# alpha-davidson/TensorBNN

Measured on AMD Instinct MI355X. Metric: leapfrog steps/sec (whole node), higher is better.
Workload: dtype f32

## Files before the change

### tensorbnn_amd/csrc/kernels_fast3.hpp

```cpp
#pragma once
#include <type_traits>
#include "kernels_fast.hpp"

template <int I, int N, class F>
__device__ __forceinline__ void sfor3(F&& f) {
    if constexpr (I < N) { f(std::integral_constant<int, I>{}); sfor3<I + 1, N>(f); }
}
template <class S>
struct F3Cfg : FastCfg<S> {
    using B = FastCfg<S>;
    static constexpr int NF(int l) { return (B::out(l) % 16 == 1 || B::out(l) % 16 == 2) ? B::out(l) % 16 : 0; }
    static constexpr int MTF(int l) { return NF(l) ? B::MT(l) - 1 : B::MT(l); }
    static constexpr int fslot(int l, int f) { return 16 * MTF(l) + 4 * f; }
    static constexpr int funit(int l, int f) { return 16 * MTF(l) + f; }
    static constexpr int NLM3 = MTF(B::NL - 1) == 0 ? B::NL - 1 : B::NL;
    static_assert(NLM3 == B::NLM, "fast3 expects the same MFMA/VALU split of the last layer as fast");
    static constexpr int dw_tiles_plain() { int o = 0; for (int m = 0; m < NLM3; ++m) o += MTF(m) * B::NT(m); return o; }
    static constexpr bool NCF(int l) {
        return dw_tiles_plain() <= 39 && l < NLM3 && B::NT(l) >= 2 && MTF(l) >= 1 && MTF(l) <= 4 && B::in(l) + 1 - 16 * (B::NT(l) - 1) <= 4;
    }
    static constexpr int NTF(int l) { return NCF(l) ? B::NT(l) - 1 : B::NT(l); }
    static constexpr int dwt3(int l) { return MTF(l) * NTF(l) + (NCF(l) ? 2 : 0); }
    static constexpr int dwoff3(int l) { int o = 0; for (int m = 0; m < l && m < NLM3; ++m) o += dwt3(m); return o; }
    static constexpr int dwfr3(int l) { return dwoff3(l) + MTF(l) * NTF(l); }
// ... 1066 lines not shown
    static constexpr bool ENABLED = C::DW3_TILES > 0 && C::EP3_TILES == C::DW3_TILES && C::P() >= 2048 &&
                                    (size_t)DENSE_OFF + P4 <= (size_t)C::LDS3_FLOATS;

    template <int W>
    static constexpr int coop_index(int t) {
        if (!CO::ENABLED) return -1;
        for (int l = 0; l < C::NLM3; ++l)
            if (C::MTF(l) > 0 && W < C::MTF(l))
                for (int nt = 0; nt < C::NTF(l); ++nt)
                    if (t == C::dwoff3(l) + W * C::NTF(l) + nt) return CO::cwoff(l) + nt;
        return -1;
    }

    template <int W, int t = 0>
    static __device__ __forceinline__ void stage(f32x4* st, f32x4 (&own)[KMAX], const f32x4 (&dW)[T], const f32x4 (&dWc)[CO::DWC], int lane) {
        if constexpr (t < C::DW3_TILES) {
            f32x4 v = dW[t];
            constexpr int ci = coop_index<W>(t);
            if constexpr (ci >= 0) v += dWc[ci];
            constexpr int sl = slot(t, W);
            if constexpr (sl >= 0) st[sl * 64 + lane] = v;
            else own[t / FAST_WAVES] = v;
            stage<W, t + 1>(st, own, dW, dWc, lane);
        }
    }
    template <int W, int l = 0>
    static __device__ __forceinline__ void stage_nf_coop(f32x4* st, const f32x4 (&dWc)[CO::DWC], int lane) {
        if constexpr (CO::ENABLED && l < C::NLM3) {
            if constexpr (C::MTF(l) > 0 && W < C::MTF(l) && C::NCF(l)) {
                const int i16 = lane & 15, g = lane >> 4;
                if ((i16 & 3) == 0) st[slot(C::dwfr3(l), W) * 64 + 16 * W + 4 * g + (i16 >> 2)] += dWc[CO::cwoff(l) + C::NTF(l)];
            }
            stage_nf_coop<W, l + 1>(st, dWc, lane);
        }
    }
    template <int W, int t, int c>
    static __device__ __forceinline__ f32x4 cpy(const f32x4* st, const f32x4 (&own)[KMAX], int lane) {
        constexpr int sl = slot(t, c);
        if constexpr (sl >= 0) return st[sl * 64 + lane];
        else return own[t / FAST_WAVES];
    }
    static constexpr int NLd = C::NLM3 > 0 ? C::NLM3 : 1;
    template <int W, int k = 0>
    static __device__ __forceinline__ void tiles_sum(const f32x4* st, const f32x4 (&own)[KMAX], int lane, f32x4 (&sum)[KMAX]) {
        if constexpr (k < KMAX) {
            constexpr int t = FAST_WAVES * k + W;
            if constexpr (t < C::DW3_TILES && nf_index(t < C::DW3_TILES ? t : 0) < 0) {
                const f32x4 c0 = cpy<W, t, 0>(st, own, lane), c1 = cpy<W, t, 1>(st, own, lane), c2 = cpy<W, t, 2>(st, own, lane), c3 = cpy<W, t, 3>(st, own, lane);
                sum[k] = (c0 + c1) + (c2 + c3);
            }
            tiles_sum<W, k + 1>(st, own, lane, sum);
        }
    }
    template <int W, int l = 0>
    static __device__ __forceinline__ void nf_sum(const f32x4* st, const f32x4 (&own)[KMAX], int lane, f32x4 (&nfs)[NLd]) {
        if constexpr (l < C::NLM3) {
            if constexpr (C::NCF(l) && (C::dwfr3(l) & (FAST_WAVES - 1)) == W) {
                constexpr int t = C::dwfr3(l);
                const f32x4 c0 = cpy<W, t, 0>(st, own, lane) + cpy<W, t + 1, 0>(st, own, lane), c1 = cpy<W, t, 1>(st, own, lane) + cpy<W, t + 1, 1>(st, own, lane),
                            c2 = cpy<W, t, 2>(st, own, lane) + cpy<W, t + 1, 2>(st, own, lane), c3 = cpy<W, t, 3>(st, own, lane) + cpy<W, t + 1, 3>(st, own, lane);
                nfs[l] = (c0 + c1) + (c2 + c3);
            }
            nf_sum<W, l + 1>(st, own, lane, nfs);
        }
    }
    template <int W, int l = 0>
    static __device__ __forceinline__ void tiles_out(float* dense, const f32x4 (&sum)[KMAX], const f32x4 (&nfs)[NLd], int lane) {
        if constexpr (l < C::NLM3) {
            constexpr int in = C::in(l), out = C::out(l), MT = C::MTF(l);
            if constexpr (C::NCF(l) && (C::dwfr3(l) & (FAST_WAVES - 1)) == W) {
                const int b = lane >> 2, col = unit_of(in, 16 * (C::NT(l) - 1) + 4 * (lane & 3), true);
                if (b < 4 * MT && col >= 0) {
#pragma unroll
                    for (int r = 0; r < 4; ++r) {
                        const int row = unit_of(out, 4 * b + r, false);
                        if (row >= 0) dense[C::offW(l) + (col < in ? row * in + col : in * out + row)] = nfs[l][r];
                    }
                }
            }
            tiles_out_full<W, l, 0>(dense, sum, lane);
            tiles_out<W, l + 1>(dense, sum, nfs, lane);
        }
    }
    template <int W, int l, int k>
    static __device__ __forceinline__ void tiles_out_full(float* dense, const f32x4 (&sum)[KMAX], int lane) {
        constexpr int in = C::in(l), out = C::out(l), MT = C::MTF(l), NT = C::NTF(l);
        if constexpr (k < MT * NT) {
            constexpr int t = C::dwoff3(l) + k, mt = k / (NT > 0 ? NT : 1), nt = k % (NT > 0 ? NT : 1);
            if constexpr ((t & (FAST_WAVES - 1)) == W) {
                const int cs = 16 * nt + (lane & 15), row0 = 16 * mt + 4 * (lane >> 4);
                const int col = l == 0 ? (cs <= in ? cs : -1) : unit_of(in, cs, true);
                if (col >= 0) {
#pragma unroll
                    for (int r = 0; r < 4; ++r) {
                        const int row = unit_of(out, row0 + r, false);
                        if (row >= 0) dense[C::offW(l) + (col < in ? row * in + col : in * out + row)] = sum[t / FAST_WAVES][r];
                    }
                }
            }
            tiles_out_full<W, l, k + 1>(dense, sum, lane);
        }
    }

    template <int W>
    static __device__ __forceinline__ void run(float* __restrict__ lds, float* __restrict__ slab, const f32x4 (&dW)[T], const f32x4 (&dWc)[CO::DWC],
                                               const float (&FP)[FPd], int tid, int lane) {
        const int i16 = lane & 15, g = lane >> 4;
        f32x4* st = reinterpret_cast<f32x4*>(lds);
        float* lb = lds + ST_FLOATS;
        float* dense = lds + DENSE_OFF;
        f32x4 own[KMAX];
        __syncthreads();
        stage<W>(st, own, dW, dWc, lane);
        stage_nf_coop<W>(st, dWc, lane);
        {
            int o = (W * C::FP_REGS * 4 + g) * 16 + i16;
            asm volatile("" : "+v"(o));
#pragma unroll
            for (int r = 0; r < C::FP_REGS; ++r) lb[o + r * 64] = FP[r];
        }
        if (tid < P4 - C::P()) dense[C::P() + tid] = 0.f;
        __syncthreads();
        TSTAMPO(63);
        f32x4 sum[KMAX], nfs[NLd];
        tiles_sum<W>(st, own, lane, sum);
        nf_sum<W>(st, own, lane, nfs);
        float fv[FringeVals<S, 0>::total()];
        int fd[FringeVals<S, 0>::total()];
        FringeVals<S, 0>::template run<0>(lb, tid, fv, fd);
        TSTAMPO(35);
        tiles_out<W>(dense, sum, nfs, lane);
#pragma unroll
        for (int i = 0; i < FringeVals<S, 0>::total(); ++i) if (fd[i] >= 0) dense[fd[i]] = fv[i];
        TSTAMPO(36);
        __syncthreads();
        TSTAMPO(37);
        {
            constexpr int N4 = P4 / 4, NE = (N4 + FAST_THREADS - 1) / FAST_THREADS;
            f32x4 d[NE];
#pragma unroll
            for (int k = 0; k < NE; ++k) {
                const int e = tid + k * FAST_THREADS;
                d[k] = *reinterpret_cast<const f32x4*>(dense + 4 * (e < N4 ? e : 0));
            }
#pragma unroll
            for (int k = 0; k < NE; ++k) {
                const int e = tid + k * FAST_THREADS;
                if (e < N4) store16<true>(slab + 4 * e, d[k]);
            }
        }
    }
};

__device__ __forceinline__ void lds_dma16(const float* gsrc, float* lbase) {
#if defined(__HIP_DEVICE_COMPILE__)
    __builtin_amdgcn_global_load_lds(gsrc, lbase, 16, 0, 0);
#else
    (void)gsrc; (void)lbase;
#endif
}

template <class S>
__global__ __launch_bounds__(FAST_THREADS, 1) __attribute__((amdgpu_waves_per_eu(1, 1))) void k_fwd_bwd_fast3(
    NetDev nd, const float* __restrict__ qimg, const float* __restrict__ eta,
    const float* __restrict__ X, const float* __restrict__ Y, long n,
    float* __restrict__ slabs, int pitch, double* __restrict__ pstat, unsigned long long* __restrict__ stamps, ChainStride cs)
{
    using C = F3Cfg<S>;
    if (chain_done(cs.ctl, cs.t, blockIdx.y)) return;
    qimg += (size_t)blockIdx.y * cs.img; eta += (size_t)blockIdx.y * cs.eta; slabs += (size_t)blockIdx.y * cs.slab; pstat += (size_t)blockIdx.y * PSTAT_CAP;
    static_assert(C::VL && C::NF(C::NL - 1) == C::out(C::NL - 1) && C::MTF(C::NL - 1) == 0, "fast3: last layer must be all-fringe");
    using CO = Coop3<S>;
    static_assert((C::LDS3_FLOATS + (CO::ENABLED ? 2 * CO::XB : 4)) * 4 + 64 <= 160 * 1024, "LDS budget");
    static_assert((size_t)FAST_WAVES * C::FP_REGS * 64 <= (size_t)C::LDS3_FLOATS, "fringe staging does not fit");
#define TB_STAMP(i) do { if (stamps && threadIdx.x == 0 && blockIdx.x == 0) { stamps[i] = wall_clock64(); stamps[8 + i] = clock64(); } } while (0)
    TB_STAMP(0); TSTAMPO(57);
    __shared__ __attribute__((aligned(16))) float lds[C::LDS3_FLOATS];
    __shared__ __attribute__((aligned(16))) float xch[CO::ENABLED ? 2 * CO::XB : 4];
    __shared__ double red[FAST_WAVES];
    const int tid = threadIdx.x, lane = tid & 63, wave = __builtin_amdgcn_readfirstlane(tid >> 6);
    const int i16 = lane & 15, g = lane >> 4;
    float* wl = lds + C::STATIC_FLOATS + wave * C::WAVE3_FLOATS;
    constexpr int d_in = C::in(0), d_out = C::out(C::NL - 1), L = C::NL - 1;
    const long ntiles = (n + 15) / 16;
    const long W = (long)gridDim.x * FAST_WAVES;
    const long wg = (long)blockIdx.x * FAST_WAVES + wave;
    float xn[C::KS0], yn[d_out], wn = 1.f;
    auto fetch = [&](long tile) {
        const long row = tile * 16 + i16;
        const bool ok = tile < ntiles && row < n;
#pragma unroll
        for (int t = 0; t < C::KS0; ++t) {
            const int u = 4 * t + g;
            xn[t] = (ok && u < d_in) ? X[row * d_in + u] : 0.f;
        }
#pragma unroll
        for (int o = 0; o < d_out; ++o) yn[o] = ok ? Y[row * d_out + o] : 0.f;
        wn = row_weight<S>(Y, n, row, ok);
    };
    long main_end = ntiles;
    int ncoop = 0;
    if constexpr (CO::ENABLED) {
        const long G = gridDim.x, rem = ntiles % W;
        if (rem > 0 && rem <= 2 * G) { main_end = ntiles - rem; ncoop = rem <= G ? 1 : 2; }
    }
    if constexpr ((TBNN_SKEL & 1) != 0) { main_end = 0; ncoop = 0; }
    float xc[2][C::KS0], yc[2][d_out], wc[2];
#pragma unroll
    for (int j = 0; j < 2; ++j) {
        const long ct = main_end + (long)j * gridDim.x + blockIdx.x;
        const long row = ct * 16 + i16;
        const bool ok = CO::ENABLED && j < ncoop && ct < ntiles && row < n;
#pragma unroll
        for (int t = 0; t < C::KS0; ++t) {
            const int u = 4 * t + g;
            xc[j][t] = (ok && u < d_in) ? X[row * d_in + u] : 0.f;
        }
#pragma unroll
        for (int o = 0; o < d_out; ++o) yc[j][o] = ok ? Y[row * d_out + o] : 0.f;
        wc[j] = row_weight<S>(Y, n, row, ok);
    }
    long tile = wg;
    fetch(tile);
    constexpr bool WTDMA = C::STATIC_FLOATS > C::WB_FLOATS;
    if constexpr (WTDMA) {
        constexpr int WT = C::STATIC_FLOATS - C::WB_FLOATS, NCHUNK = (WT + 255) / 256;
        static_assert(C::WB_FLOATS % 4 == 0 && WT % 4 == 0, "16-B pieces");
        for (int c = wave; c < NCHUNK; c += FAST_WAVES) {
            const int off = C::WB_FLOATS + c * 256;
            if (c * 256 + lane * 4 < WT) lds_dma16(qimg + off + lane * 4, lds + off);
        }
    }
    {
        constexpr int N4 = (WTDMA ? C::WB_FLOATS : C::STATIC_FLOATS) / 4, IT = (N4 + FAST_THREADS - 1) / FAST_THREADS;
        const float4* src = reinterpret_cast<const float4*>(qimg);
        float4* dst = reinterpret_cast<float4*>(lds);
        float4 v[IT];
#pragma unroll
        for (int k = 0; k < IT; ++k) { const int e = tid + k * FAST_THREADS; v[k] = e < N4 ? src[e] : make_float4(0.f, 0.f, 0.f, 0.f); }
        __builtin_amdgcn_sched_barrier(0);
        float4* z = reinterpret_cast<float4*>(wl);
        for (int e = lane; e < C::WAVE3_FLOATS / 4; e += 64) z[e] = make_float4(0.f, 0.f, 0.f, 0.f);
        __builtin_amdgcn_sched_barrier(0);
#pragma unroll
        for (int k = 0; k < IT; ++k) { const int e = tid + k * FAST_THREADS; if (e < N4) dst[e] = v[k]; }
    }
    __syncthreads();
    TB_STAMP(1); TSTAMPO(58);

    constexpr int NFd = C::maxNF() > 0 ? C::maxNF() : 1;
    f32x4 dW[C::DW3_TILES > 0 ? C::DW3_TILES : 1];
#pragma unroll
    for (int t = 0; t < C::DW3_TILES; ++t) dW[t] = f32x4{0.f, 0.f, 0.f, 0.f};
    float FP[C::FP_REGS > 0 ? C::FP_REGS : 1];
#pragma unroll
    for (int t = 0; t < C::FP_REGS; ++t) FP[t] = 0.f;
    const float sigma = lik_sigma(nd, eta);
    const float inv_var = lik_inv_var<S>(nd, sigma);
    const float np1 = lik_np1<S>(nd);
    double stat = 0.0;

    if (g == 0) wl[C::aoff3(0) + d_in * C::PR + i16] = 1.f;
#pragma unroll
    for (int l = 1; l < C::NLM3; ++l)
        if (C::in(l) % 16 == 0 && g == 0) wl[C::aoff3(l) + C::in(l) * C::PR + i16] = 1.f;
    typename Fwd3<S, 0>::Pre P0;
    Fwd3<S, 0>::pre_all(P0, lds, i16, g);

    bool first = true;
    bool wt_pending = WTDMA;
    if (WTDMA && !((long)blockIdx.x * FAST_WAVES + FAST_WAVES - 1 < main_end)) {
        asm volatile("s_waitcnt vmcnt(0)" ::: "memory");
        __syncthreads();
        wt_pending = false;
    }
    for (; tile < main_end; tile += W) {
        Tile3<S> T;
        float y[d_out];
        const bool rvalid = tile * 16 + i16 < n;
#pragma unroll
        for (int t = 0; t < C::KS0; ++t) {
            T.x0[t] = xn[t];
            const int u = 4 * t + g;
            if (u < d_in) wl[C::aoff3(0) + u * C::PR + i16] = xn[t];
        }
#pragma unroll
        for (int o = 0; o < d_out; ++o) y[o] = yn[o];
        const float wt = wn;
        fetch(tile + W);
        TSTAMP(0);
        Fwd3<S, 0>::run_h(T, lds, wl, i16, g, P0);
        if (wt_pending) {
            asm volatile("s_waitcnt vmcnt(0)" ::: "memory");
            __syncthreads();
            wt_pending = false;
        }
        float dzf[NFd];
#pragma unroll
        for (int o = 0; o < d_out; ++o) dzf[o] = rvalid ? lik_delta<S>(T.af[L][o], y[o], inv_var, g == 0, stat, wt, np1) : 0.f;
        TSTAMP(30);
        if constexpr (!C::NCF(L > 0 ? L - 1 : 0)) FringeDW<S, L>::run(FP, T, dzf, g);
        f32x4 dzL[C::MT(L)];
        f32x4 dzp[C::MT(L - 1)];
        float dzpf[NFd];
        Bwd3<S, L>::da(T, lds, i16, g, dzL, dzf, dzp, dzpf);
        TSTAMP(31);
        {
            constexpr int LM = L - 1;
            float Aop[Bwd3<S, LM>::MTd][4], Bop[C::NT(LM)][4], Fop[8];
            typename Bwd3<S, LM>::NFOps NFop;
            Bwd3<S, LM>::issue(dzp, dzpf, wl, i16, g, Aop, Bop, Fop);
            Bwd3<S, LM>::nf_load(NFop, wl, lane);
            if constexpr (C::NCF(LM)) FringeDW<S, L>::run(FP, T, dzf, g);
            TSTAMP(32);
            FringeDW<S, LM>::run(FP, T, dzpf, g);
            Bwd3<S, LM>::nf_mfma(dW, NFop);
            TSTAMP(33);
            if constexpr (LM > 0) {
                f32x4 dzq[C::MT(LM - 1)];
                float dzqf[NFd];
                Bwd3<S, LM>::da(T, lds, i16, g, dzp, dzpf, dzq, dzqf);
                SCHED_FENCE();
                TSTAMP(34);
                Pipe3<S, LM - 1>::run(dW, FP, T, lds, wl, i16, g, dzq, dzqf, Aop, Bop, Fop);
            } else {
                Bwd3<S, 0>::dw(dW, Aop, Bop);
                Bwd3<S, 0>::fdw(FP, Fop, Bop);
            }
        }
        if (first) { TB_STAMP(2); TSTAMPO(59); first = false; }
    }
    TB_STAMP(3); TSTAMPO(60);
    mfma_drain_acc(dW);
    f32x4 dWc[CO::DWC];
#pragma unroll
    for (int t = 0; t < CO::DWC; ++t) dWc[t] = f32x4{0.f, 0.f, 0.f, 0.f};
    if constexpr (CO::ENABLED) {
        if constexpr (C::P() >= 1024) {
            const long ct0 = main_end + blockIdx.x, ct1 = ct0 + gridDim.x;
            if (ncoop > 0 && ct0 < ntiles) CO::tile(dWc, FP, stat, lds, wl, xch, wave, lane, i16, g, inv_var, np1, xc[0], yc[0], ct0 * 16 + i16 < n, wc[0]);
            if (ncoop > 1 && ct1 < ntiles) {
                CO::tile(dWc, FP, stat, lds, wl, xch, wave, lane, i16, g, inv_var, np1, xc[1], yc[1], ct1 * 16 + i16 < n, wc[1]);
            }
        } else {
#pragma unroll 1
            for (int j = 0; j < ncoop; ++j) {
                const long ct = main_end + (long)j * gridDim.x + blockIdx.x;
                if (ct >= ntiles) break;
                float xj[C::KS0], yj[d_out];
#pragma unroll
                for (int t = 0; t < C::KS0; ++t) xj[t] = j == 0 ? xc[0][t] : xc[1][t];
#pragma unroll
                for (int o = 0; o < d_out; ++o) yj[o] = j == 0 ? yc[0][o] : yc[1][o];
                CO::tile(dWc, FP, stat, lds, wl, xch, wave, lane, i16, g, inv_var, np1, xj, yj, ct * 16 + i16 < n, j == 0 ? wc[0] : wc[1]);
            }
        }
    }
    TB_STAMP(5); TSTAMPO(62);

    if constexpr (Epi3<S>::ENABLED) {
        float* slab = slabs + (size_t)blockIdx.x * pitch;
        switch (wave) {
            case 0: Epi3<S>::template run<0>(lds, slab, dW, dWc, FP, tid, lane); break;
            case 1: Epi3<S>::template run<1>(lds, slab, dW, dWc, FP, tid, lane); break;
            case 2: Epi3<S>::template run<2>(lds, slab, dW, dWc, FP, tid, lane); break;
            default: Epi3<S>::template run<3>(lds, slab, dW, dWc, FP, tid, lane); break;
        }
        const double wtot = wave_sum_lane0(stat);
        if (lane == 0) red[wave] = wtot;
        __syncthreads();
        if (tid == 0) {
            double t = 0.0;
            for (int w = 0; w < FAST_WAVES; ++w) t += red[w];
            pstat[blockIdx.x] = t;
        }
    } else {
        const double wtot = wave_sum_lane0(stat);
        if (lane == 0) red[wave] = wtot;
        float* slab = slabs + (size_t)blockIdx.x * pitch;
        constexpr bool ONE_PASS = C::DW3_TILES > 0 && C::EP3_TILES == C::DW3_TILES &&
                                  (size_t)FAST_WAVES * (C::DW3_TILES * 256 + C::FP_REGS * 64) <= (size_t)C::LDS3_FLOATS;
        if constexpr (ONE_PASS) {
            float* lb = lds + FAST_WAVES * C::DW3_TILES * 256;
            TSTAMP(20);
            __syncthreads();
            TSTAMP(21);
            f32x4* mine = reinterpret_cast<f32x4*>(lds) + wave * (C::DW3_TILES * 64);
#pragma unroll
            for (int t = 0; t < C::DW3_TILES; ++t) mine[t * 64 + lane] = dW[t];
            TSTAMP(22);
            if constexpr (CO::ENABLED) { if (ncoop > 0) CO::template merge<0>(mine, dWc, wave, lane, 0, C::DW3_TILES); }
            TSTAMP(23);
#pragma unroll
            for (int r = 0; r < C::FP_REGS; ++r) lb[((size_t)(wave * C::FP_REGS + r) * 4 + g) * 16 + i16] = FP[r];
            TSTAMP(24);
            __syncthreads();
            TB_STAMP(6); TSTAMPO(63);
            SlabOut3<S, 0>::run(lds, slab, wave, lane, 0, C::DW3_TILES);
            TB_STAMP(7);
            FringeOut<S, 0>::run(lb, slab, tid);
// ... 75 lines not shown
```

### tensorbnn_amd/csrc/kernels_hmc.hpp

```cpp
#pragma once
#include "common.hpp"
#include "update_ops.hpp"

template <int UC = UPD_COLS, int UG = UPD_GROUPS>
__global__ __launch_bounds__(UC * UG) void k_update(
    NetDev nd, int mode, float eps, const float* __restrict__ eta,
    const float* __restrict__ slabs, int nslab, int pitch,
    const float* __restrict__ q_cur, const float* __restrict__ g_cur,
    float* __restrict__ q, float* __restrict__ p, float* __restrict__ g,
    const int* __restrict__ imgmap, float* __restrict__ qimg, float* __restrict__ gd = nullptr, int img_floats = 0,
    const StepCtl* __restrict__ ctl = nullptr, int t = 0)
{
    if (ctl && mode != UPD_GRAD_ONLY) {
        const StepCtl me = ctl[blockIdx.y];
        eps = me.eps;
        if (t == 0) mode = UPD_FIRST;
        else if (t < me.L) mode = UPD_MID;
        else if (t == me.L) mode = UPD_LAST;
        else return;
    }
    if (blockIdx.y) {
        const size_t c = blockIdx.y, cp = c * (size_t)nd.P;
        eta += c * nd.H; slabs += c * (size_t)nslab * pitch;
        q_cur += cp; g_cur += cp; q += cp; p += cp; g += cp;
        if (qimg) qimg += c * (size_t)img_floats;
        if (gd) gd += cp;
    }
    __shared__ float4 part[UG][UC];
    const int tx = threadIdx.x, ty = threadIdx.y;
    const int c4 = blockIdx.x * UC + tx;
    const int jf = c4 * 4 + ty;
    const bool fin = ty < 4 && jf < nd.P;
    UpdPre u;
    if (fin) upd_prefetch(u, nd, mode, eta, jf, q_cur, g_cur, q, p, imgmap);
    float4 gs = make_float4(0.f, 0.f, 0.f, 0.f);
    if (mode != UPD_FIRST) {
        part[ty][tx] = upd_column_partial<UG>(slabs, nslab, pitch, c4, ty);
        __syncthreads();
#pragma unroll
        for (int h = UG / 2; h > 0; h >>= 1) {
            if (ty < h) {
                const float4 a = part[ty][tx], b = part[ty + h][tx];
                part[ty][tx] = make_float4(a.x + b.x, a.y + b.y, a.z + b.z, a.w + b.w);
            }
            __syncthreads();
        }
        gs = part[0][tx];
    }
    if (!fin) return;
    const float gj = ty == 0 ? gs.x : ty == 1 ? gs.y : ty == 2 ? gs.z : gs.w;
    upd_finish(u, nd, mode, eps, eta, jf, gj, q, p, g, imgmap, qimg, gd);
}

__global__ __launch_bounds__(256) void k_slab_reduce(const float* __restrict__ slabs, int nslab, int pitch, int P,
                                                      float* __restrict__ out, double* __restrict__ outd = nullptr) {
    __shared__ float part[4][64];
    const int x = threadIdx.x, y = threadIdx.y, j = blockIdx.x * 64 + x;
    float s0 = 0.f, s1 = 0.f, s2 = 0.f, s3 = 0.f;
    if (j < P) {
        const float* src = slabs + j;
        int w = y;
        for (; w + 12 < nslab; w += 16) {
            s0 += src[(size_t)w * pitch]; s1 += src[(size_t)(w + 4) * pitch];
            s2 += src[(size_t)(w + 8) * pitch]; s3 += src[(size_t)(w + 12) * pitch];
        }
        for (; w < nslab; w += 4) s0 += src[(size_t)w * pitch];
    }
    part[y][x] = (s0 + s1) + (s2 + s3);
    __syncthreads();
    if (y == 0 && j < P) {
        const float v = (part[0][x] + part[1][x]) + (part[2][x] + part[3][x]);
        if (out) out[j] = v;
        if (outd) outd[j] = (double)v;
    }
}

__global__ __launch_bounds__(256) void k_shard_pack(int P, const float* __restrict__ row, const double* __restrict__ pstat, int nstat,
                                                     double* __restrict__ buf, double sub) {
    __shared__ double red[4];
    const int j = blockIdx.x * blockDim.x + threadIdx.x;
    if (row && j < P) buf[j] = (double)row[j];
    if (blockIdx.x == 0) {
        double st = 0.0;
        for (int w = threadIdx.x; w < nstat; w += blockDim.x) st += pstat[w];
        st = block_sum(st, red);
        if (threadIdx.x == 0) buf[P] = st - sub;
    }
}
__global__ __launch_bounds__(256) void k_shard_unpack(int P, const double* __restrict__ buf, float* __restrict__ row,
                                                       double* __restrict__ stat_red) {
    const int j = blockIdx.x * blockDim.x + threadIdx.x;
    if (j < P) row[j] = (float)buf[j];
    if (j == 0) stat_red[0] = buf[P];
}

#define LIKC_BLOCKS 64
__global__ __launch_bounds__(256) void k_pois_const(const float* __restrict__ Y, const float* __restrict__ w, long n, int d_out,
                                                     double* __restrict__ out, double r) {
    __shared__ double red[4];
    double c = 0.0, bad = 0.0;
    const long nel = n * d_out;
    const double lgr = r > 0.0 ? lgamma(r) : 0.0;
    for (long el = (long)blockIdx.x * 256 + threadIdx.x; el < nel; el += (long)LIKC_BLOCKS * 256) {
        const float y = Y[el];
        if (!(y >= 0.f && y < INFINITY)) { bad += 1.0; continue; }
        const double wt = w ? (double)w[el / d_out] : 1.0;
        double t = lgamma((double)y + 1.0);
        if (r > 0.0) t += lgr - lgamma((double)y + r);
        c += wt * t;
    }
    c = block_sum(c, red);
    bad = block_sum(bad, red);
    if (threadIdx.x == 0) { out[2 * blockIdx.x] = c; out[2 * blockIdx.x + 1] = bad; }
}

__global__ __launch_bounds__(256) void k_copy_f32(int n, const float* __restrict__ src, float* __restrict__ dst) {
    const int j = blockIdx.x * blockDim.x + threadIdx.x;
    if (j < n) dst[j] = src[j];
}

__global__ __launch_bounds__(256) void k_make_image(int P, const float* __restrict__ q,
                                                    const int* __restrict__ imgmap, float* __restrict__ qimg,
                                                    long q_stride = 0, long img_stride = 0) {
    q += (size_t)blockIdx.y * q_stride; qimg += (size_t)blockIdx.y * img_stride;
    const int j = blockIdx.x * blockDim.x + threadIdx.x;
    if (j < P) { const float v = q[j]; qimg[imgmap[j]] = v; const int m1 = imgmap[P + j]; if (m1 >= 0) qimg[m1] = v; }
}

__device__ __forceinline__ double data_logp(const NetDev& nd, const float* __restrict__ eta, double stat, double n, double lik_c) {
    if (nd.lik == TBNN_LIK_POISSON) return stat - lik_c;
    if (nd.lik == TBNN_LIK_NEG_BINOMIAL) return stat - lik_c;
    if (nd.lik == TBNN_LIK_BERNOULLI || nd.lik == TBNN_LIK_CATEGORICAL) return stat;
    if (nd.lik == TBNN_LIK_STUDENT_T) {
        const double nu = (double)nd.lik_df, s = (double)lik_sigma(nd, eta);
        const double c = lgamma(0.5 * (nu + 1.0)) - lgamma(0.5 * nu) - 0.5 * log(nu * 3.14159265358979323846) - log(s);
        return n * (double)nd.d_out * c - 0.5 * (nu + 1.0) * stat;
    }
    const double s = (double)lik_sigma(nd, eta);
    const double nel = (double)n * (double)nd.d_out;
    return -0.5 * (2.0 * nel * log(s) + stat / (s * s) + nel * 1.8378770664093453 );
}

__device__ __forceinline__ double prior_logp_partial(const NetDev& nd, const float* __restrict__ eta,
                                                     const float* __restrict__ q) {
    double acc = 0.0;
    for (int l = 0; l < nd.nl; ++l) {
        for (int part = 0; part < 2; ++part) {
            const int off = part ? nd.offB[l] : nd.offW[l];
            const int cnt = part ? nd.out[l] : nd.out[l] * nd.in[l];
            const float loc = eta[4 * l + 2 * part];
            const float gg = eta[4 * l + 2 * part + 1];
            const float scale = gg * gg;
            if (nd.prior[l] == TBNN_PRIOR_CAUCHY) {
                const float lb = logf(3.14159265358979323846f * scale);
                for (int e = threadIdx.x; e < cnt; e += blockDim.x) {
                    const float z = (q[off + e] - loc) / scale;
                    acc += (double)(logf(1.f + z * z) - lb);
                }
            } else {
                const float s = fminf(fmaxf(scale, 1e-8f), 1e8f);
                for (int e = threadIdx.x; e < cnt; e += blockDim.x) {
                    const float d = (q[off + e] - loc) / s;
                    acc += -0.5 * (double)(d * d);
                }
                if (threadIdx.x == 0) acc += -0.5 * (2.0 * (double)logf(s) + 1.8378770664093453);
            }
        }
    }
    return acc;
}

__global__ __launch_bounds__(1024) void k_begin(
    NetDev nd, const float* __restrict__ p0_inj, const float* __restrict__ logu_inj,
    uint32_t epoch, uint32_t key0, uint32_t key1, float* __restrict__ p, Scal* __restrict__ sc, uint32_t seed_hi = 0)
{
    __shared__ double red[16];
    if (blockIdx.y) {
        const uint32_t c = blockIdx.y;
        key1 = (((key1 ^ seed_hi) + c) ^ seed_hi);
        p += (size_t)c * nd.P; sc += c;
        if (p0_inj) p0_inj += (size_t)c * nd.P;
        if (logu_inj) logu_inj += c;
    }
    double k = 0.0;
    if (p0_inj) {
        for (int j = threadIdx.x; j < nd.P; j += blockDim.x) { const float v = p0_inj[j]; p[j] = v; k += (double)v * (double)v; }
    } else {
        for (int b = threadIdx.x; 4 * b < nd.P; b += blockDim.x) {
            float v[4];
            philox_normal4((uint32_t)b, epoch, PURPOSE_MOMENTUM, key0, key1, v);
#pragma unroll
            for (int i = 0; i < 4; ++i)
                if (4 * b + i < nd.P) { p[4 * b + i] = v[i]; k += (double)v[i] * (double)v[i]; }
        }
    }
    k = block_sum(k, red);
    if (threadIdx.x == 0) {
        sc->k0 = 0.5 * k;
        sc->logu = logu_inj ? (double)logu_inj[0] : (double)philox_logu(epoch, PURPOSE_LOGU, key0, key1);
    }
}

enum { EN_CUR = 0, EN_NEW = 1, EN_TRACE = 2, EN_REFRESH = 3 };
// ... 117 lines not shown
```

### tensorbnn_amd/csrc/kernels_optim.hpp

```cpp
#pragma once
#include "common.hpp"
#include "update_ops.hpp"
#include "kernels_hmc.hpp"

struct OptChain {
    double best;
    int best_step;
    int better;
    int frozen;
    int pad;
};
struct OptStep { float a_t, r_t, b1, b2, omb1, omb2, epsilon; int amsgrad; };

__global__ __launch_bounds__(1024) void k_optim_logp(
    NetDev nd, int likelihood_only, const float* __restrict__ eta, const float* __restrict__ q,
    const double* __restrict__ partial_stat, int nslab, double n, double lik_c,
    OptChain* __restrict__ oc, int step, double* __restrict__ trace, int n_checks, int k)
{
    __shared__ double red[16];
    if (blockIdx.y) {
        const size_t c = blockIdx.y;
        eta += c * nd.H; q += c * (size_t)nd.P; partial_stat += c * PSTAT_CAP; oc += c;
        trace += c * (size_t)n_checks;
    }
    double st = 0.0;
    for (int w = threadIdx.x; w < nslab; w += blockDim.x) st += partial_stat[w];
    st = block_sum(st, red);
    double pr = 0.0;
    if (!likelihood_only) {
        pr = prior_logp_partial(nd, eta, q);
        pr = block_sum(pr, red);
    }
    if (threadIdx.x != 0) return;
    const double lp = pr + data_logp(nd, eta, st, n, lik_c);
    trace[k] = lp;
    const bool fin = isfinite(lp);
    const bool better = fin && lp > oc->best;
    oc->better = better ? 1 : 0;
    if (better) { oc->best = lp; oc->best_step = step; }
    if (!fin) oc->frozen = 1;
}

template <int UC = UPD_COLS, int UG = UPD_GROUPS>
__global__ __launch_bounds__(UC * UG) void k_optim(
    NetDev nd, int likelihood_only, OptStep s, int checked, const float* __restrict__ eta,
    const float* __restrict__ slabs, int nslab, int pitch,
    float* __restrict__ q, float* __restrict__ g, float* __restrict__ m, float* __restrict__ v, float* __restrict__ vhat,
    float* __restrict__ q_best, const OptChain* __restrict__ oc,
    const int* __restrict__ imgmap, float* __restrict__ qimg, int img_floats)
{
    if (blockIdx.y) {
        const size_t c = blockIdx.y, cp = c * (size_t)nd.P;
        eta += c * nd.H; slabs += c * (size_t)nslab * pitch;
        q += cp; g += cp; m += cp; v += cp; vhat += cp; q_best += cp; oc += c;
        if (qimg) qimg += c * (size_t)img_floats;
    }
    const int better = checked ? oc->better : 0, frozen = oc->frozen;
    __shared__ float4 part[UG][UC];
    const int tx = threadIdx.x, ty = threadIdx.y;
    const int c4 = blockIdx.x * UC + tx;
    const int jf = c4 * 4 + ty;
    const bool fin = ty < 4 && jf < nd.P;
    float th = 0.f, mj = 0.f, vj = 0.f, vh = 0.f, loc = 0.f, scale = 1.f;
    int prior = 0, m0 = -1, m1 = -1;
    if (fin) {
        th = q[jf];
        if (better) q_best[jf] = th;
        if (!frozen) {
            if (!likelihood_only) prior_params(nd, eta, jf, prior, loc, scale);
            mj = m[jf]; vj = v[jf]; vh = vhat[jf];
            if (imgmap) { m0 = imgmap[jf]; m1 = imgmap[nd.P + jf]; }
        }
    }
    if (frozen) return;
    part[ty][tx] = upd_column_partial<UG>(slabs, nslab, pitch, c4, ty);
    __syncthreads();
#pragma unroll
    for (int h = UG / 2; h > 0; h >>= 1) {
        if (ty < h) {
            const float4 a = part[ty][tx], b = part[ty + h][tx];
            part[ty][tx] = make_float4(a.x + b.x, a.y + b.y, a.z + b.z, a.w + b.w);
        }
        __syncthreads();
    }
    if (!fin) return;
    const float4 gs = part[0][tx];
    float gj = ty == 0 ? gs.x : ty == 1 ? gs.y : ty == 2 ? gs.z : gs.w;
    if (!likelihood_only) gj += prior_grad(prior, loc, scale, th);
    g[jf] = gj;
    mj = s.b1 * mj + s.omb1 * gj;
    vj = s.b2 * vj + s.omb2 * (gj * gj);
    vh = s.amsgrad ? fmaxf(vh, vj) : vj;
    th += s.a_t * mj / (sqrtf(vh) * s.r_t + s.epsilon);
    m[jf] = mj; v[jf] = vj; vhat[jf] = vh; q[jf] = th;
    if (imgmap) { qimg[m0] = th; if (m1 >= 0) qimg[m1] = th; }
}

__global__ __launch_bounds__(256) void k_optim_finish(int P, int keep_best, const OptChain* __restrict__ oc, const float* __restrict__ q,
                                                      float* __restrict__ q_best, float* __restrict__ q_cur) {
    const size_t c = blockIdx.y, cp = c * (size_t)P;
    const int j = blockIdx.x * blockDim.x + threadIdx.x;
    if (j >= P) return;
    const OptChain me = oc[c];
    const float th = q[cp + j];
    float qb = q_best[cp + j];
    if (me.better) { qb = th; q_best[cp + j] = th; }
    q_cur[cp + j] = (keep_best || me.frozen) ? qb : th;
}

__global__ __launch_bounds__(256) void k_optim_reset(int P, int chains, const float* __restrict__ q_cur, float* __restrict__ m, float* __restrict__ v,
                                                     float* __restrict__ vhat, float* __restrict__ g, float* __restrict__ q_best, OptChain* __restrict__ oc) {
    const size_t c = blockIdx.y, cp = c * (size_t)P;
    const int j = blockIdx.x * blockDim.x + threadIdx.x;
    if (j < P) { m[cp + j] = 0.f; v[cp + j] = 0.f; vhat[cp + j] = 0.f; g[cp + j] = 0.f; q_best[cp + j] = q_cur[cp + j]; }
    if (j == 0) { OptChain z; z.best = -INFINITY; z.best_step = 0; z.better = 0; z.frozen = 0; z.pad = 0; oc[c] = z; }
}
```

### tensorbnn_amd/csrc/update_ops.hpp

```cpp
#pragma once
#include "common.hpp"

enum { UPD_GRAD_ONLY = 0, UPD_FIRST = 1, UPD_MID = 2, UPD_LAST = 3 };

__device__ __forceinline__ void prior_params(const NetDev& nd, const float* __restrict__ eta, int j,
                                             int& prior, float& loc, float& scale) {
    int l = 0;
#pragma unroll 1
    for (int m = 1; m < nd.nl; ++m) if (j >= nd.offW[m]) l = m;
    const bool isb = j >= nd.offB[l];
    prior = nd.prior[l];
    loc = eta[4 * l + (isb ? 2 : 0)];
    const float g = eta[4 * l + (isb ? 3 : 1)];
    scale = g * g;
}

__device__ __forceinline__ float prior_grad(int prior, float loc, float scale, float x) {
    if (prior == TBNN_PRIOR_CAUCHY) {
        const float z = (x - loc) / scale;
        return 2.f * z / (scale * (1.f + z * z));
    }
    const float s = fminf(fmaxf(scale, 1e-8f), 1e8f);
    return -(x - loc) / (s * s);
}

#ifndef UPD_COLS
#define UPD_COLS 16
#endif
#ifndef UPD_GROUPS
#define UPD_GROUPS 32
#endif
#define UPD_BIG_P 8192
#define UPD_COLS_BIG 32
#define UPD_GROUPS_BIG 16

struct UpdPre {
    float q_j = 0.f, p_j = 0.f, gc_j = 0.f, qc_j = 0.f, loc = 0.f, scale = 1.f;
    int prior = 0, m0 = -1, m1 = -1;
};
__device__ __forceinline__ void upd_prefetch(UpdPre& u, const NetDev& nd, int mode, const float* __restrict__ eta, int jf,
                                             const float* __restrict__ q_cur, const float* __restrict__ g_cur,
                                             const float* __restrict__ q, const float* __restrict__ p, const int* __restrict__ imgmap) {
    if (mode != UPD_FIRST) { prior_params(nd, eta, jf, u.prior, u.loc, u.scale); u.q_j = q[jf]; }
    if (mode == UPD_FIRST) { u.gc_j = g_cur[jf]; u.qc_j = q_cur[jf]; }
    if (mode != UPD_GRAD_ONLY) u.p_j = p[jf];
    if (imgmap && (mode == UPD_FIRST || mode == UPD_MID)) { u.m0 = imgmap[jf]; u.m1 = imgmap[nd.P + jf]; }
}
template <int UPD_GROUPS_T = UPD_GROUPS>
__device__ __forceinline__ float4 upd_column_partial(const float* slabs, int nslab, int pitch, int c4, int ty) {
    constexpr int UG = UPD_GROUPS_T;
    float4 z = make_float4(0.f, 0.f, 0.f, 0.f);
    float4 s0 = z, s1 = z, s2 = z, s3 = z;
    if (c4 * 4 < pitch) {
        const float4* base = reinterpret_cast<const float4*>(slabs) + c4;
        const int p4 = pitch >> 2;
        int w = ty;
        for (; w + 7 * UG < nslab; w += 8 * UG) {
            float4 v[8];
#pragma unroll
            for (int k = 0; k < 8; ++k) v[k] = base[(size_t)(w + k * UG) * p4];
#pragma unroll
            for (int k = 0; k < 8; k += 4) {
                s0.x += v[k].x; s0.y += v[k].y; s0.z += v[k].z; s0.w += v[k].w;
                s1.x += v[k + 1].x; s1.y += v[k + 1].y; s1.z += v[k + 1].z; s1.w += v[k + 1].w;
                s2.x += v[k + 2].x; s2.y += v[k + 2].y; s2.z += v[k + 2].z; s2.w += v[k + 2].w;
                s3.x += v[k + 3].x; s3.y += v[k + 3].y; s3.z += v[k + 3].z; s3.w += v[k + 3].w;
            }
        }
        for (; w < nslab; w += UG) {
            const float4 a = base[(size_t)w * p4];
            s0.x += a.x; s0.y += a.y; s0.z += a.z; s0.w += a.w;
        }
    }
    float4 s;
    s.x = (s0.x + s1.x) + (s2.x + s3.x); s.y = (s0.y + s1.y) + (s2.y + s3.y);
    s.z = (s0.z + s1.z) + (s2.z + s3.z); s.w = (s0.w + s1.w) + (s2.w + s3.w);
    return s;
}
__device__ __forceinline__ void upd_finish(const UpdPre& u, const NetDev& nd, int mode, float eps, const float* __restrict__ eta, int j,
                                           float gj, float* __restrict__ q, float* __restrict__ p, float* __restrict__ g,
                                           const int* __restrict__ imgmap, float* __restrict__ qimg, float* __restrict__ gd) {
    if (mode != UPD_FIRST && mode != UPD_MID && gd) {
        const float sg = nd.lik == TBNN_LIK_GAUSSIAN ? lik_sigma(nd, eta) : 1.f;
        gd[j] = gj * (sg * sg);
    }
    if (mode != UPD_FIRST) gj += prior_grad(u.prior, u.loc, u.scale, u.q_j);
    if (mode == UPD_GRAD_ONLY) { g[j] = gj; return; }
    if (mode == UPD_FIRST) {
        const float pj = u.p_j + 0.5f * eps * u.gc_j;
        const float qj = u.qc_j + eps * pj;
        p[j] = pj; q[j] = qj;
        if (imgmap) { qimg[u.m0] = qj; if (u.m1 >= 0) qimg[u.m1] = qj; }
        return;
    }
    float pj = u.p_j + eps * gj;
    if (mode == UPD_MID) {
        const float qj = u.q_j + eps * pj;
        p[j] = pj; q[j] = qj;
        if (imgmap) { qimg[u.m0] = qj; if (u.m1 >= 0) qimg[u.m1] = qj; }
    } else {
        g[j] = gj;
        pj = pj - 0.5f * eps * gj;
        p[j] = pj;
    }
}
```

Measured before the change: 20990.

## Overlap prologue loads with LDS init and streamline update-kernel reductions

The fast3 kernel prologue is reordered so the weight-image global loads are issued right after the first tile fetch. The LDS zeroing and image store then happen before the DMA tail and the coop-tile loads, and the DMA uses inline asm that sets m0 directly. The update kernel issues its first batch of slab-column loads before the prior-parameter prefetch. It replaces the barrier-per-step tree reduction with one barrier followed by per-thread register summation over the shared column. Prior lookup becomes a branchless unrolled select over layers, and asm barriers pin values into registers. The aim is to cut prologue and update-kernel latency, at the cost of hand-written m0 asm, extra registers and more redundant LDS reads per thread.

```diff
diff --git a/tensorbnn_amd/csrc/kernels_fast3.hpp b/tensorbnn_amd/csrc/kernels_fast3.hpp
--- a/tensorbnn_amd/csrc/kernels_fast3.hpp
+++ b/tensorbnn_amd/csrc/kernels_fast3.hpp
@@ -1242,11 +1242,18 @@
     }
 };
 
-__device__ __forceinline__ void lds_dma16(const float* gsrc, float* lbase) {
+__device__ __forceinline__ void lds_dma16_unseen(const float* gsrc, float* lbase) {
 #if defined(__HIP_DEVICE_COMPILE__)
-    __builtin_amdgcn_global_load_lds(gsrc, lbase, 16, 0, 0);
+    unsigned keep;
+    asm volatile("s_mov_b32 %0, m0\n\ts_mov_b32 m0, %2\n\ts_nop 0\n\tglobal_load_lds_dwordx4 %1, off\n\ts_mov_b32 m0, %0"
+                 : "=&s"(keep) : "v"(gsrc), "s"((unsigned)(size_t)lbase) : "memory");
 #else
     (void)gsrc; (void)lbase;
+#endif
+}
+__device__ __forceinline__ void wait_vmem_all() {
+#if defined(__HIP_DEVICE_COMPILE__)
+    __builtin_amdgcn_s_waitcnt(0x0F70);
 #endif
 }
 
@@ -1257,6 +1264,7 @@
     float* __restrict__ slabs, int pitch, double* __restrict__ pstat, unsigned long long* __restrict__ stamps, ChainStride cs)
 {
     using C = F3Cfg<S>;
+    asm volatile("" :: "s"(cs.ctl), "s"(cs.t), "s"(cs.img), "s"(stamps), "s"(qimg), "s"(X), "s"(Y), "s"(n), "s"(gridDim.x));
     if (chain_done(cs.ctl, cs.t, blockIdx.y)) return;
     qimg += (size_t)blockIdx.y * cs.img; eta += (size_t)blockIdx.y * cs.eta; slabs += (size_t)blockIdx.y * cs.slab; pstat += (size_t)blockIdx.y * PSTAT_CAP;
     static_assert(C::VL && C::NF(C::NL - 1) == C::out(C::NL - 1) && C::MTF(C::NL - 1) == 0, "fast3: last layer must be all-fringe");
@@ -1288,6 +1296,16 @@
         for (int o = 0; o < d_out; ++o) yn[o] = ok ? Y[row * d_out + o] : 0.f;
         wn = row_weight<S>(Y, n, row, ok);
     };
+    long tile = wg;
+    fetch(tile);
+    constexpr bool WTDMA = C::STATIC_FLOATS > C::WB_FLOATS;
+    constexpr int IMG_N4 = (WTDMA ? C::WB_FLOATS : C::STATIC_FLOATS) / 4, IMG_IT = (IMG_N4 + FAST_THREADS - 1) / FAST_THREADS;
+    f32x4 imgv[IMG_IT];
+#pragma unroll
+    for (int k = 0; k < IMG_IT; ++k) {
+        const int e = tid + k * FAST_THREADS;
+        imgv[k] = *reinterpret_cast<const f32x4*>(qimg + 4 * (e < IMG_N4 ? e : 0));
+    }
     long main_end = ntiles;
     int ncoop = 0;
     if constexpr (CO::ENABLED) {
@@ -1295,47 +1313,39 @@
         if (rem > 0 && rem <= 2 * G) { main_end = ntiles - rem; ncoop = rem <= G ? 1 : 2; }
     }
     if constexpr ((TBNN_SKEL & 1) != 0) { main_end = 0; ncoop = 0; }
-    float xc[2][C::KS0], yc[2][d_out], wc[2];
-#pragma unroll
-    for (int j = 0; j < 2; ++j) {
-        const long ct = main_end + (long)j * gridDim.x + blockIdx.x;
-        const long row = ct * 16 + i16;
-        const bool ok = CO::ENABLED && j < ncoop && ct < ntiles && row < n;
-#pragma unroll
-        for (int t = 0; t < C::KS0; ++t) {
-            const int u = 4 * t + g;
-            xc[j][t] = (ok && u < d_in) ? X[row * d_in + u] : 0.f;
-        }
-#pragma unroll
-        for (int o = 0; o < d_out; ++o) yc[j][o] = ok ? Y[row * d_out + o] : 0.f;
-        wc[j] = row_weight<S>(Y, n, row, ok);
-    }
-    long tile = wg;
-    fetch(tile);
-    constexpr bool WTDMA = C::STATIC_FLOATS > C::WB_FLOATS;
+    {
+        __builtin_amdgcn_sched_barrier(0);
+        float4* z = reinterpret_cast<float4*>(wl);
+        for (int e = lane; e < C::WAVE3_FLOATS / 4; e += 64) z[e] = make_float4(0.f, 0.f, 0.f, 0.f);
+        __builtin_amdgcn_sched_barrier(0);
+#pragma unroll
+        for (int k = 0; k < IMG_IT; ++k) { const int e = tid + k * FAST_THREADS; if (e < IMG_N4) *reinterpret_cast<f32x4*>(lds + 4 * e) = imgv[k]; }
+        wait_vmem_all();
+    }
+    __syncthreads();
     if constexpr (WTDMA) {
         constexpr int WT = C::STATIC_FLOATS - C::WB_FLOATS, NCHUNK = (WT + 255) / 256;
         static_assert(C::WB_FLOATS % 4 == 0 && WT % 4 == 0, "16-B pieces");
         for (int c = wave; c < NCHUNK; c += FAST_WAVES) {
             const int off = C::WB_FLOATS + c * 256;
-            if (c * 256 + lane * 4 < WT) lds_dma16(qimg + off + lane * 4, lds + off);
-        }
-    }
-    {
-        constexpr int N4 = (WTDMA ? C::WB_FLOATS : C::STATIC_FLOATS) / 4, IT = (N4 + FAST_THREADS - 1) / FAST_THREADS;
-        const float4* src = reinterpret_cast<const float4*>(qimg);
-        float4* dst = reinterpret_cast<float4*>(lds);
-        float4 v[IT];
-#pragma unroll
-        for (int k = 0; k < IT; ++k) { const int e = tid + k * FAST_THREADS; v[k] = e < N4 ? src[e] : make_float4(0.f, 0.f, 0.f, 0.f); }
-        __builtin_amdgcn_sched_barrier(0);
-        float4* z = reinterpret_cast<float4*>(wl);
-        for (int e = lane; e < C::WAVE3_FLOATS / 4; e += 64) z[e] = make_float4(0.f, 0.f, 0.f, 0.f);
-        __builtin_amdgcn_sched_barrier(0);
-#pragma unroll
-        for (int k = 0; k < IT; ++k) { const int e = tid + k * FAST_THREADS; if (e < N4) dst[e] = v[k]; }
-    }
-    __syncthreads();
+            if (c * 256 + lane * 4 < WT) lds_dma16_unseen(qimg + off + lane * 4, lds + off);
+        }
+    }
+    float xc[2][C::KS0], yc[2][d_out], wc[2];
+#pragma unroll
+    for (int j = 0; j < 2; ++j) {
+        const long ct = main_end + (long)j * gridDim.x + blockIdx.x;
+        const long row = ct * 16 + i16;
+        const bool ok = CO::ENABLED && j < ncoop && ct < ntiles && row < n;
+#pragma unroll
+        for (int t = 0; t < C::KS0; ++t) {
+            const int u = 4 * t + g;
+            xc[j][t] = (ok && u < d_in) ? X[row * d_in + u] : 0.f;
+        }
+#pragma unroll
+        for (int o = 0; o < d_out; ++o) yc[j][o] = ok ? Y[row * d_out + o] : 0.f;
+        wc[j] = row_weight<S>(Y, n, row, ok);
+    }
     TB_STAMP(1); TSTAMPO(58);
 
     constexpr int NFd = C::maxNF() > 0 ? C::maxNF() : 1;
diff --git a/tensorbnn_amd/csrc/kernels_hmc.hpp b/tensorbnn_amd/csrc/kernels_hmc.hpp
--- a/tensorbnn_amd/csrc/kernels_hmc.hpp
+++ b/tensorbnn_amd/csrc/kernels_hmc.hpp
@@ -11,6 +11,7 @@
     const int* __restrict__ imgmap, float* __restrict__ qimg, float* __restrict__ gd = nullptr, int img_floats = 0,
     const StepCtl* __restrict__ ctl = nullptr, int t = 0)
 {
+    asm volatile("" :: "s"(mode), "s"(ctl), "s"(slabs), "s"(nslab), "s"(pitch), "s"(eta), "s"(q), "s"(p), "s"(imgmap), "s"(nd.P), "s"(nd.nl));
     if (ctl && mode != UPD_GRAD_ONLY) {
         const StepCtl me = ctl[blockIdx.y];
         eps = me.eps;
@@ -32,23 +33,17 @@
     const int jf = c4 * 4 + ty;
     const bool fin = ty < 4 && jf < nd.P;
     UpdPre u;
+    UpdCol col;
+    if (mode != UPD_FIRST) upd_column_issue<UG>(col, slabs, nslab, pitch, c4, ty);
     if (fin) upd_prefetch(u, nd, mode, eta, jf, q_cur, g_cur, q, p, imgmap);
-    float4 gs = make_float4(0.f, 0.f, 0.f, 0.f);
+    float gj = 0.f;
     if (mode != UPD_FIRST) {
-        part[ty][tx] = upd_column_partial<UG>(slabs, nslab, pitch, c4, ty);
+        part[ty][tx] = upd_column_sum<UG>(col, slabs, nslab, pitch, c4, ty);
         __syncthreads();
-#pragma unroll
-        for (int h = UG / 2; h > 0; h >>= 1) {
-            if (ty < h) {
-                const float4 a = part[ty][tx], b = part[ty + h][tx];
-                part[ty][tx] = make_float4(a.x + b.x, a.y + b.y, a.z + b.z, a.w + b.w);
-            }
-            __syncthreads();
-        }
-        gs = part[0][tx];
+        if (!fin) return;
+        gj = upd_block_sum<UC, UG>(part, tx, ty);
     }
     if (!fin) return;
-    const float gj = ty == 0 ? gs.x : ty == 1 ? gs.y : ty == 2 ? gs.z : gs.w;
     upd_finish(u, nd, mode, eps, eta, jf, gj, q, p, g, imgmap, qimg, gd);
 }
 
diff --git a/tensorbnn_amd/csrc/kernels_optim.hpp b/tensorbnn_amd/csrc/kernels_optim.hpp
--- a/tensorbnn_amd/csrc/kernels_optim.hpp
+++ b/tensorbnn_amd/csrc/kernels_optim.hpp
@@ -75,17 +75,8 @@
     if (frozen) return;
     part[ty][tx] = upd_column_partial<UG>(slabs, nslab, pitch, c4, ty);
     __syncthreads();
-#pragma unroll
-    for (int h = UG / 2; h > 0; h >>= 1) {
-        if (ty < h) {
-            const float4 a = part[ty][tx], b = part[ty + h][tx];
-            part[ty][tx] = make_float4(a.x + b.x, a.y + b.y, a.z + b.z, a.w + b.w);
-        }
-        __syncthreads();
-    }
     if (!fin) return;
-    const float4 gs = part[0][tx];
-    float gj = ty == 0 ? gs.x : ty == 1 ? gs.y : ty == 2 ? gs.z : gs.w;
+    float gj = upd_block_sum<UC, UG>(part, tx, ty);
     if (!likelihood_only) gj += prior_grad(prior, loc, scale, th);
     g[jf] = gj;
     mj = s.b1 * mj + s.omb1 * gj;
diff --git a/tensorbnn_amd/csrc/update_ops.hpp b/tensorbnn_amd/csrc/update_ops.hpp
--- a/tensorbnn_amd/csrc/update_ops.hpp
+++ b/tensorbnn_amd/csrc/update_ops.hpp
@@ -3,15 +3,23 @@
 
 enum { UPD_GRAD_ONLY = 0, UPD_FIRST = 1, UPD_MID = 2, UPD_LAST = 3 };
 
+__device__ __forceinline__ void prior_fetch(const NetDev& nd, const float* __restrict__ eta, int j,
+                                            int& prior, float& loc, float& g) {
+    int l = 0, ob = nd.offB[0], pr = nd.prior[0];
+#pragma unroll
+    for (int m = 1; m < TBNN_MAX_LAYERS; ++m) {
+        const bool in = m < nd.nl && j >= nd.offW[m];
+        l = in ? m : l; ob = in ? nd.offB[m] : ob; pr = in ? nd.prior[m] : pr;
+    }
+    const bool isb = j >= ob;
+    prior = pr;
+    loc = eta[4 * l + (isb ? 2 : 0)];
+    g = eta[4 * l + (isb ? 3 : 1)];
+}
 __device__ __forceinline__ void prior_params(const NetDev& nd, const float* __restrict__ eta, int j,
                                              int& prior, float& loc, float& scale) {
-    int l = 0;
-#pragma unroll 1
-    for (int m = 1; m < nd.nl; ++m) if (j >= nd.offW[m]) l = m;
-    const bool isb = j >= nd.offB[l];
-    prior = nd.prior[l];
-    loc = eta[4 * l + (isb ? 2 : 0)];
-    const float g = eta[4 * l + (isb ? 3 : 1)];
+    float g;
+    prior_fetch(nd, eta, j, prior, loc, g);
     scale = g * g;
 }
 
@@ -35,19 +43,34 @@
 #define UPD_GROUPS_BIG 16
 
 struct UpdPre {
-    float q_j = 0.f, p_j = 0.f, gc_j = 0.f, qc_j = 0.f, loc = 0.f, scale = 1.f;
+    float q_j = 0.f, p_j = 0.f, gc_j = 0.f, qc_j = 0.f, loc = 0.f, sroot = 1.f;
     int prior = 0, m0 = -1, m1 = -1;
 };
 __device__ __forceinline__ void upd_prefetch(UpdPre& u, const NetDev& nd, int mode, const float* __restrict__ eta, int jf,
                                              const float* __restrict__ q_cur, const float* __restrict__ g_cur,
                                              const float* __restrict__ q, const float* __restrict__ p, const int* __restrict__ imgmap) {
-    if (mode != UPD_FIRST) { prior_params(nd, eta, jf, u.prior, u.loc, u.scale); u.q_j = q[jf]; }
+    if (mode != UPD_FIRST) { prior_fetch(nd, eta, jf, u.prior, u.loc, u.sroot); u.q_j = q[jf]; }
     if (mode == UPD_FIRST) { u.gc_j = g_cur[jf]; u.qc_j = q_cur[jf]; }
     if (mode != UPD_GRAD_ONLY) u.p_j = p[jf];
     if (imgmap && (mode == UPD_FIRST || mode == UPD_MID)) { u.m0 = imgmap[jf]; u.m1 = imgmap[nd.P + jf]; }
 }
+struct UpdCol {
+    float4 v[8];
+    bool first;
+};
 template <int UPD_GROUPS_T = UPD_GROUPS>
-__device__ __forceinline__ float4 upd_column_partial(const float* slabs, int nslab, int pitch, int c4, int ty) {
+__device__ __forceinline__ void upd_column_issue(UpdCol& c, const float* slabs, int nslab, int pitch, int c4, int ty) {
+    constexpr int UG = UPD_GROUPS_T;
+    c.first = c4 * 4 < pitch && ty + 7 * UG < nslab;
+    if (c.first) {
+        const float4* base = reinterpret_cast<const float4*>(slabs) + c4;
+        const int p4 = pitch >> 2;
+#pragma unroll
+        for (int k = 0; k < 8; ++k) c.v[k] = base[(size_t)(ty + k * UG) * p4];
+    }
+}
+template <int UPD_GROUPS_T = UPD_GROUPS>
+__device__ __forceinline__ float4 upd_column_sum(const UpdCol& c, const float* slabs, int nslab, int pitch, int c4, int ty) {
     constexpr int UG = UPD_GROUPS_T;
     float4 z = make_float4(0.f, 0.f, 0.f, 0.f);
     float4 s0 = z, s1 = z, s2 = z, s3 = z;
@@ -55,6 +78,22 @@
         const float4* base = reinterpret_cast<const float4*>(slabs) + c4;
         const int p4 = pitch >> 2;
         int w = ty;
+        if (c.first) {
+            float4 v[8];
+#pragma unroll
+            for (int k = 0; k < 8; ++k) {
+                v[k] = c.v[k];
+                asm volatile("" : "+v"(v[k].x), "+v"(v[k].y), "+v"(v[k].z), "+v"(v[k].w));
+            }
+#pragma unroll
+            for (int k = 0; k < 8; k += 4) {
+                s0.x += v[k].x; s0.y += v[k].y; s0.z += v[k].z; s0.w += v[k].w;
+                s1.x += v[k + 1].x; s1.y += v[k + 1].y; s1.z += v[k + 1].z; s1.w += v[k + 1].w;
+                s2.x += v[k + 2].x; s2.y += v[k + 2].y; s2.z += v[k + 2].z; s2.w += v[k + 2].w;
+                s3.x += v[k + 3].x; s3.y += v[k + 3].y; s3.z += v[k + 3].z; s3.w += v[k + 3].w;
+            }
+            w += 8 * UG;
+        }
         for (; w + 7 * UG < nslab; w += 8 * UG) {
             float4 v[8];
 #pragma unroll
@@ -77,6 +116,25 @@
     s.z = (s0.z + s1.z) + (s2.z + s3.z); s.w = (s0.w + s1.w) + (s2.w + s3.w);
     return s;
 }
+template <int UPD_GROUPS_T = UPD_GROUPS>
+__device__ __forceinline__ float4 upd_column_partial(const float* slabs, int nslab, int pitch, int c4, int ty) {
+    UpdCol c;
+    upd_column_issue<UPD_GROUPS_T>(c, slabs, nslab, pitch, c4, ty);
+    return upd_column_sum<UPD_GROUPS_T>(c, slabs, nslab, pitch, c4, ty);
+}
+template <int UC, int UG>
+__device__ __forceinline__ float upd_block_sum(const float4 (&part)[UG][UC], int tx, int ty) {
+    const float* col = reinterpret_cast<const float*>(&part[0][0]) + 4 * tx + ty;
+    float t[UG];
+#pragma unroll
+    for (int i = 0; i < UG; ++i) t[i] = col[i * UC * 4];
+#pragma unroll
+    for (int h = UG / 2; h > 0; h >>= 1) {
+#pragma unroll
+        for (int i = 0; i < h; ++i) t[i] = t[i] + t[i + h];
+    }
+    return t[0];
+}
 __device__ __forceinline__ void upd_finish(const UpdPre& u, const NetDev& nd, int mode, float eps, const float* __restrict__ eta, int j,
                                            float gj, float* __restrict__ q, float* __restrict__ p, float* __restrict__ g,
                                            const int* __restrict__ imgmap, float* __restrict__ qimg, float* __restrict__ gd) {
@@ -84,20 +142,23 @@
         const float sg = nd.lik == TBNN_LIK_GAUSSIAN ? lik_sigma(nd, eta) : 1.f;
         gd[j] = gj * (sg * sg);
     }
-    if (mode != UPD_FIRST) gj += prior_grad(u.prior, u.loc, u.scale, u.q_j);
+    float sroot = u.sroot;
+    int m0 = u.m0, m1 = u.m1;
+    asm volatile("" : "+v"(sroot), "+v"(m0), "+v"(m1));
+    if (mode != UPD_FIRST) gj += prior_grad(u.prior, u.loc, sroot * sroot, u.q_j);
     if (mode == UPD_GRAD_ONLY) { g[j] = gj; return; }
     if (mode == UPD_FIRST) {
         const float pj = u.p_j + 0.5f * eps * u.gc_j;
         const float qj = u.qc_j + eps * pj;
         p[j] = pj; q[j] = qj;
-        if (imgmap) { qimg[u.m0] = qj; if (u.m1 >= 0) qimg[u.m1] = qj; }
+        if (imgmap) { qimg[m0] = qj; if (m1 >= 0) qimg[m1] = qj; }
         return;
     }
     float pj = u.p_j + eps * gj;
     if (mode == UPD_MID) {
         const float qj = u.q_j + eps * pj;
         p[j] = pj; q[j] = qj;
-        if (imgmap) { qimg[u.m0] = qj; if (u.m1 >= 0) qimg[u.m1] = qj; }
+        if (imgmap) { qimg[m0] = qj; if (m1 >= 0) qimg[m1] = qj; }
     } else {
         g[j] = gj;
         pj = pj - 0.5f * eps * gj;
```

Result: faster. 21690, median of 6 (+3.3%).
